# kelseyicotton/rawaudiovae_kelsey

Hardware: AMD Instinct MI355X
Metric: audio frames/sec (fwd+bwd+step), 1024-sample frames (higher is better)
Workload: dtype bf16; 1 GPU; C2 raw-audio VAE train step: S=1024 H=2048 L=64, per-GPU batch 4096, kl_beta=1e-4, Adam lr=1e-4; global_batch=4096, parallelism=dp1, launch=eager, wgrad_slabs=fp16

## Files before the change

rawaudiovae_kelsey_amd/csrc/gemm_bf16.h:

```cpp
#pragma once
#include <type_traits>

#include "common.h"
#include "philox.h"

namespace rv {

enum : int {
  EPI_BIAS_ACT_BF16 = 0,
  EPI_F32 = 1,
  EPI_TANH_LOSS = 2,
  EPI_MASK_BF16 = 3,
  EPI_REPARAM = 4,
  EPI_REPARAM_BWD = 5,
};

struct GemmArgs {
  const bf16_t* A;
  const bf16_t* B;
  long lda, ldb;
  int k_tiles;
  int tiles_m, tiles_n;
  int splits;
  int M_valid, N_valid;
  int relu;
  float* out_f32;
  long ld_f32, split_stride_f32;
  void* out_f16;
  float* f16_unscale;
  long us_ld, us_split_stride;
  bf16_t* out_bf16;
  long ld_bf16;
  const float* bias;
  const bf16_t* mask;
  long ld_mask;
  int mask_fp8;
  const float* x;
  long ld_x;
// ... 20 lines not shown
  float* eps_out;
  unsigned long long seed;
  const long long* step_counter;
  float* mulv;
  bf16_t* z;
  float* kl_partial;
  const float* eps;
  float kl_beta, inv_nk;
  const float* dmu_ext;
  const float* dlv_ext;
  bf16_t* dmulv;
  float* dbh_partial;
  int wt;
};

template <int ROWS>
__device__ __forceinline__ int swz_mn(int k) {
  if constexpr (ROWS >= 128)
    return (k & 3) | (((k >> 3) & 1) << 2);
  else
    return ((k >> 1) & 1) | (((k >> 3) & 1) << 1);
}

__device__ __forceinline__ int swz_mn8(int k) { return ((k >> 1) & 3) | (((k >> 4) & 1) << 2); }

template <int ROWS, bool KMAJ, int NW, bool F8MN = false>
struct StageOffsets {
  static constexpr int NINSTR = ROWS * 128 / 1024;
  static constexpr int PER_WAVE = NINSTR / NW;
  static_assert(NINSTR % NW == 0, "tile must split evenly over the waves");
// ... 119 lines not shown
  }
}

__device__ __forceinline__ unsigned long long pack_fp8x8(const float (&v)[8]) {
  float c[8];
#pragma unroll
  for (int e = 0; e < 8; ++e) c[e] = fminf(fmaxf(v[e], -448.f), 448.f);
  unsigned lo = 0, hi = 0;
  lo = __builtin_amdgcn_cvt_pk_fp8_f32(c[0], c[1], lo, false);
  lo = __builtin_amdgcn_cvt_pk_fp8_f32(c[2], c[3], lo, true);
  hi = __builtin_amdgcn_cvt_pk_fp8_f32(c[4], c[5], hi, false);
  hi = __builtin_amdgcn_cvt_pk_fp8_f32(c[6], c[7], hi, true);
  return ((unsigned long long)hi << 32) | lo;
}

template <int GL>
__device__ __forceinline__ void wait_tiles_in_flight(int tiles) {
  if (tiles >= 6) asm volatile("s_waitcnt vmcnt(%0)" ::"n"(6 * GL < 63 ? 6 * GL : 63) : "memory");
  else if (tiles == 5) asm volatile("s_waitcnt vmcnt(%0)" ::"n"(5 * GL < 63 ? 5 * GL : 63) : "memory");
  else if (tiles == 4) asm volatile("s_waitcnt vmcnt(%0)" ::"n"(4 * GL < 63 ? 4 * GL : 63) : "memory");
  else if (tiles == 3) asm volatile("s_waitcnt vmcnt(%0)" ::"n"(3 * GL) : "memory");
  else if (tiles == 2) asm volatile("s_waitcnt vmcnt(%0)" ::"n"(2 * GL) : "memory");
  else if (tiles == 1) asm volatile("s_waitcnt vmcnt(%0)" ::"n"(GL) : "memory");
  else asm volatile("s_waitcnt vmcnt(0)" ::: "memory");
}

template <int NW>
__device__ __forceinline__ float block_sum(float v, float* red) {
  v = wave_sum(v);
  const int lane = threadIdx.x & 63, w = threadIdx.x >> 6;
  if (lane == 0) red[w] = v;
  __syncthreads();
  float r = 0.f;
  if (threadIdx.x == 0)
    for (int i = 0; i < NW; ++i) r += red[i];
  __syncthreads();
  return r;
}

struct NoGather {};
template <bool A_KMAJ, bool B_KMAJ, bool FP8, typename Hook, typename BRows = NoGather>
__device__ __forceinline__ void mainloop_pingpong(const bf16_t* __restrict__ Ag, const bf16_t* __restrict__ Bg,
                                                  const long lda, const long ldb, const int nk, lds_char* smem,
                                                  const int wave, const int lane, f32x4 (&acc)[8][4], Hook tail_hook,
                                                  BRows b_rows = BRows{}, const long b_half_gather = 0,
                                                  const bf16_t* __restrict__ Ag_next = nullptr,
                                                  const bf16_t* __restrict__ Bg_next = nullptr, const bool resumed = false) {
  constexpr bool GATHER_B = !std::is_same<BRows, NoGather>::value;
  const bool has_next = Ag_next != nullptr;
  constexpr int HALF = 128 * 128;
  constexpr int BUF = 4 * HALF;
  const int wr = wave >> 2, wc = wave & 3;
  StageOffsets<128, A_KMAJ, 8, FP8 && !A_KMAJ> sa;
  StageOffsets<128, B_KMAJ, 8, FP8 && !B_KMAJ> sb;
  sa.init(lda, wave, lane);
  if constexpr (GATHER_B) sb.init_rows(b_rows, wave, lane);
  else sb.init(ldb, wave, lane);
  const int unit_scale = 0x7F7F7F7F;
  constexpr int KROWS = FP8 ? 128 : 64;
  constexpr int MNH = FP8 ? 64 : 128;
// ... 79 lines not shown
      if (kt + 1 < nk || has_next) asm volatile("s_waitcnt vmcnt(4)" ::: "memory");
    }
    mma(I1{}, I1{}, b1);
    if constexpr (EARLY_B) {
      if (kt + 1 < nk) rd_b(bn, nxt, 0);
    }
    stage_b(0, kt + 2);
    if (kt + 2 < nk || has_next) asm volatile("s_waitcnt vmcnt(2)" ::: "memory");
    else asm volatile("s_waitcnt vmcnt(0)" ::: "memory");
    mma(I1{}, I0{}, bq);
  };

  if (!resumed) {
    stage_a(0, 0); stage_a(1, 0); stage_b(0, 0); stage_b(1, 0);
    stage_b(0, 1);
    if (nk > 1) asm volatile("s_waitcnt vmcnt(2)" ::: "memory");
    else asm volatile("s_waitcnt vmcnt(0)" ::: "memory");
    __builtin_amdgcn_s_barrier();
  }
  if constexpr (EARLY_B) rd_b(b0, smem, 0);
  if (wr == 1) __builtin_amdgcn_s_barrier();
  __builtin_amdgcn_sched_barrier(0);

  for (int kt = 0; kt < nk; kt += 2) {
    if constexpr (EARLY_B) {
      k_tile(kt, smem, smem + BUF, b0, b2);
      k_tile(kt + 1, smem + BUF, smem, b2, b0);
    } else {
      k_tile(kt, smem, smem + BUF, b0, b0);
      k_tile(kt + 1, smem + BUF, smem, b0, b0);
    }
  }
  if (wr == 0) __builtin_amdgcn_s_barrier();
  if constexpr (FP8) asm volatile("s_nop 15\n\ts_nop 15" ::: "memory");
  __builtin_amdgcn_sched_barrier(0);
}

template <int BM, int BN, int WGM, int WGN, bool A_KMAJ, bool B_KMAJ, int EPI, int NSTAGE, bool FP8 = false>
__device__ __forceinline__ void gemm_body(const GemmArgs& p, const int bid, char* smem_generic, const int next_bid = -1,
                                          const bool resumed = false) {
  static_assert(!FP8 || NSTAGE == 8 || (A_KMAJ && B_KMAJ), "fp8 operands: K-major (forward) GEMMs on the ring loop, any layout on the ping-pong loop");
  lds_char* smem = (lds_char*)smem_generic;
  constexpr int NW = WGM * WGN;
  constexpr int A_BYTES = BM * 128, B_BYTES = BN * 128, STAGE = A_BYTES + B_BYTES;
  constexpr int B_OFF = A_BYTES;
  constexpr int WTM = BM / WGM, WTN = BN / WGN, MI = WTM / 16, NI = WTN / 16;
  constexpr int GL = STAGE / 1024 / NW;
  constexpr bool PINGPONG = NSTAGE == 8;
  static_assert(PINGPONG || (NSTAGE >= 2 && NSTAGE <= 7 && (NSTAGE - 1) * GL < 64), "vmcnt is a 6-bit counter");
  static_assert(!PINGPONG || (BM == 256 && BN == 256 && WGM == 2 && WGN == 4), "ping-pong loop: 256x256, 2x4 waves");

  const int tid = threadIdx.x, lane = tid & 63;
  const int wave = __builtin_amdgcn_readfirstlane(tid >> 6);
  const int wm = wave / WGN, wn = wave % WGN;
  const int tiles_n = p.tiles_n, nt = p.tiles_n * p.tiles_m, nwg = nt * p.splits;
  auto locate = [&](const int b_, int& split_, int& tile_m_, int& tile_n_) {
    const int xcd = b_ & 7, q = nwg >> 3, rr = nwg & 7;
    const int item = (xcd < rr ? xcd * (q + 1) : rr * (q + 1) + (xcd - rr) * q) + (b_ >> 3);
    split_ = item / nt;
    const int tid_lin = item - split_ * nt;
    if (((tiles_n | p.tiles_m) & 3) == 0) {
      const int sn = tiles_n >> 2, s4 = tid_lin >> 4, w4 = tid_lin & 15;
      tile_m_ = (s4 / sn) * 4 + (w4 >> 2);
      tile_n_ = (s4 % sn) * 4 + (w4 & 3);
    } else {
      tile_m_ = tid_lin / tiles_n;
      tile_n_ = tid_lin - tile_m_ * tiles_n;
    }
  };
  int split, tile_m, tile_n;
  locate(bid, split, tile_m, tile_n);
  const long m0 = (long)tile_m * BM, n0 = (long)tile_n * BN;
  const long k0 = (long)split * p.k_tiles * 64;
  constexpr int F8S = FP8 ? 2 : 1;
  auto a_origin = [&](const long m_, const long k_) { return A_KMAJ ? p.A + m_ * p.lda + k_ : p.A + (F8S * k_) * p.lda + m_ / F8S; };
  auto b_origin = [&](const long n_, const long k_) { return B_KMAJ ? p.B + n_ * p.ldb + k_ : p.B + (F8S * k_) * p.ldb + n_ / F8S; };
  const bf16_t* Ag = a_origin(m0, k0);
  const bf16_t* Bg = b_origin(n0, k0);
  const bf16_t *Ag_next = nullptr, *Bg_next = nullptr;
  if (next_bid >= 0) {
    int s2, tm2, tn2;
    locate(next_bid, s2, tm2, tn2);
    Ag_next = a_origin((long)tm2 * BM, (long)s2 * p.k_tiles * 64);
    Bg_next = b_origin((long)tn2 * BN, (long)s2 * p.k_tiles * 64);
  }
  const long a_step = A_KMAJ ? 64 : 64 * p.lda;
  const long b_step = B_KMAJ ? 64 : 64 * p.ldb;

  static_assert(NI % 2 == 0, "epilogue pairs column fragments");
  constexpr int NP = NI / 2;
  constexpr int CM = (EPI == EPI_REPARAM_BWD && NSTAGE == 8) ? 1 : NP >= 2 ? 2 : (MI >= 4 ? 4 : MI);
  static_assert(MI % CM == 0, "chunking must divide the wave tile");
  constexpr int CH = CM * NP;
  const int eq = lane >> 4, ej = lane & 15;
  const long colw = n0 + wn * WTN + (eq & 1) * 16 + (eq >> 1) * 8;
  const long roww = m0 + wm * WTM + ej;
  typedef int i32x4_ __attribute__((ext_vector_type(4)));

  constexpr bool PF_ROOM = !PINGPONG && MI * NI <= 16;
  constexpr bool PF_X = EPI == EPI_TANH_LOSS && PF_ROOM;
  constexpr bool PF_MASK = EPI == EPI_MASK_BF16 && PF_ROOM;
  float xpf[CH][8];
  i32x4_ mpf[CH];
  bool pf_on = false;
  if constexpr (PF_X) {
    const bool x_al0 = p.x && !p.x_hop && (p.ld_x & 3) == 0 && ((reinterpret_cast<uintptr_t>(p.x) & 15) == 0);
    if (x_al0 && m0 + BM <= p.M_valid && n0 + BN <= p.N_valid) {
      pf_on = true;
#pragma unroll
      for (int it = 0; it < CH; ++it) {
        const float* xs = p.x + (roww + 16 * (it / NP)) * p.ld_x + colw + 32 * (it % NP);
        const f32x4 lo = *(const f32x4*)xs, hi = *(const f32x4*)(xs + 4);
#pragma unroll
        for (int e = 0; e < 4; ++e) { xpf[it][e] = lo[e]; xpf[it][4 + e] = hi[e]; }
      }
    }
  }
  if constexpr (PF_MASK) {
    if (p.mask) {
      pf_on = true;
#pragma unroll
      for (int it = 0; it < CH; ++it)
        mpf[it] = *(const i32x4_*)(p.mask + (roww + 16 * (it / NP)) * p.ld_mask + colw + 32 * (it % NP));
    }
  }
  constexpr bool PF_RB = EPI == EPI_REPARAM_BWD, PF_RF = EPI == EPI_REPARAM;
  constexpr bool PF_RB_ON = PF_RB && MI == CM;
  constexpr int RF_N = MI * (NI / 2);
  f32x4 rb_m[PF_RB ? CH : 1][2], rb_l[PF_RB ? CH : 1][2], rb_e[PF_RB ? CH : (PF_RF ? RF_N : 1)][2];
  bool rb_vec[PF_RB ? CH : (PF_RF ? RF_N : 1)];
  if constexpr (PF_RB_ON) {
    const long L2p_ = 2 * p.lat_lp, L_ = p.lat_l;
    const bool al = (L_ & 3) == 0 && (reinterpret_cast<uintptr_t>(p.eps) & 15) == 0;
#pragma unroll
    for (int it = 0; it < CH; ++it) {
      const long r_ = roww + 16 * (it / NP), c_ = colw + 32 * (it % NP);
      const float* mp = p.mulv + r_ * L2p_ + c_;
      rb_m[it][0] = *(const f32x4*)mp; rb_m[it][1] = *(const f32x4*)(mp + 4);
      rb_l[it][0] = *(const f32x4*)(mp + p.lat_lp); rb_l[it][1] = *(const f32x4*)(mp + p.lat_lp + 4);
      rb_vec[it] = al && r_ < p.M_valid && c_ + 8 <= L_;
// ... 4 lines not shown
      }
    }
  }
  if constexpr (PF_RF) {
    const long L_ = p.lat_l;
    const bool al = RF_N <= 4 && p.eps_in && (L_ & 3) == 0 && (reinterpret_cast<uintptr_t>(p.eps_in) & 15) == 0;
#pragma unroll
    for (int it = 0; it < RF_N; ++it) {
      const long b_ = m0 + wm * WTM + (it / (NI / 2)) * 16 + (lane & 15);
      const long l_ = (long)tile_n * (BN / 2) + wn * (WTN / 2) + (it % (NI / 2)) * 16 + 4 * (lane >> 4);
      rb_vec[it] = al && b_ < p.M_valid && l_ + 4 <= L_;
      rb_e[it][0] = f32x4{0.f, 0.f, 0.f, 0.f};
      if (rb_vec[it]) rb_e[it][0] = *(const f32x4*)(p.eps_in + b_ * L_ + l_);
    }
  }
  if constexpr (PF_X || PF_MASK || PF_RB || PF_RF) {
    asm volatile("" ::: "memory");
    __builtin_amdgcn_sched_barrier(0);
  }

  f32x4 acc[MI][NI];
#pragma unroll
  for (int mi = 0; mi < MI; ++mi)
#pragma unroll
    for (int ni = 0; ni < NI; ++ni) acc[mi][ni] = f32x4{0.f, 0.f, 0.f, 0.f};

  constexpr bool MASK_LDS = EPI == EPI_MASK_BF16 && PINGPONG;
  static_assert(!MASK_LDS || (WTN == 64 && CH == 2 * CM), "mask through LDS: 128-byte mask rows, as many stores as DMA pieces per chunk");
  constexpr int MK_C0 = 2 * CM * 1024;
  lds_char* mk_lds = smem + wave * (WTM * 128);
  lds_char* mk_lds0 = smem + 2 * (BM + BN) * 128 + wave * MK_C0;
  bool mask_lds = false;
  const char* mk_g = nullptr;
  long mk_pitch8 = 0;
  const bool mask8 = FP8 && MASK_LDS && p.mask_fp8;
  if constexpr (MASK_LDS) {
    if (p.mask) {
      mask_lds = true;
      const int mrow = lane >> 3;
      if (mask8) {
        const int mpc = ((lane & 3) ^ (mrow & 3));
        mk_g = (const char*)p.mask + (m0 + wm * WTM + mrow) * p.ld_mask + n0 + wn * WTN + mpc * 16;
        mk_pitch8 = 8 * p.ld_mask;
      } else {
        const int mpc = (lane & 7) ^ (lane >> 3);
        mk_g = (const char*)(p.mask + (m0 + wm * WTM + mrow) * p.ld_mask + n0 + wn * WTN + mpc * 8);
        mk_pitch8 = 16 * p.ld_mask;
      }
    }
  }
  auto mask_dma = [&](int i0, int i1, lds_char* base) {
#pragma unroll
    for (int i = i0; i < i1; ++i)
      __builtin_amdgcn_global_load_lds((glb_cptr)(mk_g + (long)i * mk_pitch8),
                                       (__attribute__((address_space(3))) void*)(base + (i - i0) * 1024), 16, 0, 0);
  };
  if constexpr (PINGPONG && EPI == EPI_REPARAM) {
    static_assert(B_KMAJ && !FP8, "reparameterisation epilogue: bf16 K-major weights");
    mainloop_pingpong<A_KMAJ, B_KMAJ, FP8>(Ag, p.B + k0, p.lda, p.ldb, p.k_tiles, smem, wave, lane, acc, [&]() {},
        [&](int r) { return (((r >> 4) & 1) * p.lat_lp + (long)tile_n * (BN / 2) + (r >> 5) * 16 + (r & 15)) * p.ldb; }, 64 * p.ldb);
  } else if constexpr (PINGPONG) {
    mainloop_pingpong<A_KMAJ, B_KMAJ, FP8>(Ag, Bg, p.lda, p.ldb, p.k_tiles, smem, wave, lane, acc, [&]() {
      if constexpr (MASK_LDS) {
        if (mask_lds) mask_dma(0, 2 * CM, mk_lds0);
      }
    }, NoGather{}, 0, Ag_next, Bg_next, resumed);
  } else {
  StageOffsets<BM, A_KMAJ, NW> sa;
  StageOffsets<BN, B_KMAJ, NW> sb;
  const bf16_t* Agr = Ag;
  bool gathered = false;
  if constexpr (A_KMAJ && EPI == EPI_BIAS_ACT_BF16 && !FP8) {
    if (p.a_hop) {
      gathered = true;
      Agr = p.A + k0;
      sa.init_rows([&](int r) {
        long row = m0 + r;
        row = row < p.a_rows ? row : p.a_rows - 1;
        return (p.a_idx ? (long)p.a_idx[row] : p.a_first + row) * p.a_hop;
      }, wave, lane);
    }
    if (p.step_inc && bid == 0 && tid == 0) *p.step_inc += 1;
  }
  if (!gathered) sa.init(p.lda, wave, lane);
  const bf16_t* Bgr = Bg;
  if constexpr (EPI == EPI_REPARAM) {
    static_assert(B_KMAJ && WTN % 32 == 0, "reparameterisation epilogue: tiles of BN / 2 latents x 2 heads, wave tiles of whole (mu, logvar) fragment pairs");
    Bgr = p.B + k0;
    sb.init_rows([&](int r) { return (((r >> 4) & 1) * p.lat_lp + (long)tile_n * (BN / 2) + (r >> 5) * 16 + (r & 15)) * p.ldb; }, wave, lane);
  } else {
    sb.init(p.ldb, wave, lane);
  }
  auto copy_out = [&](int kt, const lds_char* slot_) {
    if constexpr (A_KMAJ && EPI == EPI_BIAS_ACT_BF16 && !FP8) {
      if (gathered && p.a_copy && kt % tiles_n == tile_n) {
#pragma unroll
        for (int i = 0; i < StageOffsets<BM, A_KMAJ, NW>::PER_WAVE; ++i) {
          const int t = wave + NW * i;
          const int r = 8 * t + (lane >> 3), c = (lane & 7) ^ ((r >> 1) & 7);
          const bf16x8 v_ = *(const __attribute__((address_space(3))) bf16x8*)(slot_ + t * 1024 + lane * 16);
          store_out16((bf16x8*)(p.a_copy + (m0 + r) * p.ld_copy + (long)kt * 64 + c * 8), v_, p.wt);
        }
      }
    }
  };

  const int nk = p.k_tiles;
#pragma unroll
  for (int s = 0; s < NSTAGE; ++s)
    if (s < nk) {
      sa.stage(Agr + s * a_step, smem + s * STAGE, wave);
      sb.stage(Bgr + s * b_step, smem + s * STAGE + B_OFF, wave);
    }
  wait_tiles_in_flight<GL>(nk - 1 < NSTAGE - 1 ? nk - 1 : NSTAGE - 1);
  __builtin_amdgcn_s_barrier();

  bf16x8 a0[MI], b0[NI], a1[MI], b1[NI];
#pragma unroll
  for (int mi = 0; mi < MI; ++mi) a0[mi] = load_frag<BM, A_KMAJ>(smem, wm * WTM + mi * 16, 0, lane);
#pragma unroll
  for (int ni = 0; ni < NI; ++ni) b0[ni] = load_frag<BN, B_KMAJ>(smem + B_OFF, wn * WTN + ni * 16, 0, lane);

  constexpr int NRD = MI * (A_KMAJ ? 1 : 2) + NI * (B_KMAJ ? 1 : 2);
  constexpr int NMF = MI * NI;

  auto first_half = [&](const lds_char* cur) {
#pragma unroll
    for (int mi = 0; mi < MI; ++mi) a1[mi] = load_frag<BM, A_KMAJ>(cur, wm * WTM + mi * 16, 1, lane);
#pragma unroll
// ... 562 lines not shown
        p.colsum[(long)tile_m * tiles_n * BN + n0 + tid] = s_;
      }
    }
    if constexpr (EPI == EPI_TANH_LOSS) {
      if (p.blocksum) {
        __syncthreads();
        float* red = (float*)smem_generic;
        const float s_ = block_sum<NW>(sq, red);
        if (tid == 0) p.blocksum[tile_m * tiles_n + tile_n] = s_;
      }
    }
  }
}

template <int BM, int BN, int WGM, int WGN, bool A_KMAJ, bool B_KMAJ, int EPI, int NSTAGE, bool FP8 = false>
__global__ void __launch_bounds__(64 * WGM * WGN) gemm_bf16_kernel(const GemmArgs p) {
  extern __shared__ __attribute__((aligned(16))) char smem_dyn[];
  gemm_body<BM, BN, WGM, WGN, A_KMAJ, B_KMAJ, EPI, NSTAGE, FP8>(p, blockIdx.x, smem_dyn);
}

template <bool A_KMAJ, bool B_KMAJ, int EPI>
__global__ void __launch_bounds__(512) gemm_pp_persist_kernel(const GemmArgs p) {
  static_assert(EPI == EPI_BIAS_ACT_BF16, "tile lists: epilogues that do not use LDS");
  extern __shared__ __attribute__((aligned(16))) char smem_dyn[];
  const int nwg = p.tiles_m * p.tiles_n * p.splits, G = (int)gridDim.x;
  bool resumed = false;
  for (int vb = (int)blockIdx.x; vb < nwg; vb += G) {
    gemm_body<256, 256, 2, 4, A_KMAJ, B_KMAJ, EPI, 8>(p, vb, smem_dyn, vb + G < nwg ? vb + G : -1, resumed);
    resumed = true;
  }
}

template <int BM, int BN, int WGM, int WGN, int NSTAGE, bool FP8 = false>
__global__ void __launch_bounds__(64 * WGM * WGN)
gemm_dgrad_wgrad_kernel(const GemmArgs dgrad, const GemmArgs wgrad, const int n_first) {
  extern __shared__ __attribute__((aligned(16))) char smem_dyn[];
  if ((int)blockIdx.x < n_first)
    gemm_body<BM, BN, WGM, WGN, true, false, EPI_MASK_BF16, NSTAGE, FP8>(dgrad, blockIdx.x, smem_dyn);
  else
    gemm_body<BM, BN, WGM, WGN, false, false, EPI_F32, NSTAGE, FP8>(wgrad, blockIdx.x - n_first, smem_dyn);
}

template <int BM, int BN, int WGM, int WGN, int NSTAGE, bool A1, bool B1, int E1, bool A2, bool B2, int E2>
__global__ void __launch_bounds__(64 * WGM * WGN)
gemm_dual_kernel(const GemmArgs first, const GemmArgs second, const int n_first) {
  extern __shared__ __attribute__((aligned(16))) char smem_dyn[];
  if ((int)blockIdx.x < n_first)
    gemm_body<BM, BN, WGM, WGN, A1, B1, E1, NSTAGE>(first, blockIdx.x, smem_dyn);
  else
    gemm_body<BM, BN, WGM, WGN, A2, B2, E2, NSTAGE>(second, blockIdx.x - n_first, smem_dyn);
}

}
```

rawaudiovae_kelsey_amd/csrc/gemm_launch.hip:

```cpp
#include <hip/hip_ext.h>
#include "gemm_bf16.h"
#include "adam.h"
#include "../../include/rawvae_hip.h"
#include "internal.h"

using namespace rv;

namespace rv {
thread_local int rv_store_wt = 0;
}

namespace {

int g_force_tile = -1;
int g_tile_lists = 1;

template <int BM, int BN, int WGM, int WGN, int NSTAGE, bool AK, bool BK, int EPI, bool FP8 = false>
int launch(const GemmArgs& a, long Mp, long Np, int splits, hipStream_t st) {
  constexpr int RING = NSTAGE == 8 ? 2 : NSTAGE;
  constexpr int mask_extra = (NSTAGE == 8 && EPI == EPI_MASK_BF16) ? 8 * 4096 : 0;
  constexpr int smem_max = RING * (BM + BN) * 128 + mask_extra;
  constexpr int stage_bytes = (BM + BN) * 128;
  constexpr int epi_bytes = WGM * BN * 4 + 256;
  const int used = (NSTAGE >= 8 ? RING : (a.k_tiles < RING ? a.k_tiles : RING)) * stage_bytes + mask_extra;
  const int smem = used > epi_bytes ? used : epi_bytes;
  auto kern = gemm_bf16_kernel<BM, BN, WGM, WGN, AK, BK, EPI, NSTAGE, FP8>;
  static std::atomic<unsigned long long> attr_done{0};
  lds_opt_in((const void*)kern, smem_max, attr_done);
  GemmArgs g = a;
  g.wt = rv_store_wt;
  g.tiles_m = (int)(Mp / BM);
  g.tiles_n = (int)(Np / BN);
  g.splits = splits;
  dim3 grid((unsigned)(g.tiles_m * g.tiles_n * splits), 1, 1);
  hipLaunchKernelGGL(kern, grid, dim3(64 * WGM * WGN), smem, st, g);
  RV_CHECK_LAUNCH();
  return RV_OK;
}

template <bool AK, bool BK, int EPI>
int launch_persist(const GemmArgs& a, long Mp, long Np, hipStream_t st) {
  constexpr int smem = 2 * (256 + 256) * 128;
  auto kern = gemm_pp_persist_kernel<AK, BK, EPI>;
  static std::atomic<unsigned long long> attr_done{0};
  lds_opt_in((const void*)kern, smem, attr_done);
  GemmArgs g = a;
  g.wt = rv_store_wt;
  g.tiles_m = (int)(Mp / 256);
  g.tiles_n = (int)(Np / 256);
  g.splits = 1;
// ... 34 lines not shown
    case 0: return launch<64, 64, 2, 2, 4, AK, BK, EPI>(a, Mp, Np, splits, st);
    case 1: return launch<128, 128, 2, 2, 4, AK, BK, EPI>(a, Mp, Np, splits, st);
    case 2: return launch<256, 128, 4, 2, 3, AK, BK, EPI>(a, Mp, Np, splits, st);
    case 4: return launch<128, 128, 2, 4, 4, AK, BK, EPI>(a, Mp, Np, splits, st);
    case 5: return launch<256, 256, 2, 4, 2, AK, BK, EPI>(a, Mp, Np, splits, st);
    case 7:
      if ((Kp / 64 / splits) % 2) return launch<256, 256, 2, 4, 2, AK, BK, EPI>(a, Mp, Np, splits, st);
      if constexpr (EPI == EPI_BIAS_ACT_BF16) {
        if (g_tile_lists && splits == 1 && !a.amax_part && !a.a_hop && (Mp / 256) * (Np / 256) >= 512) return launch_persist<AK, BK, EPI>(a, Mp, Np, st);
      }
      return launch<256, 256, 2, 4, 8, AK, BK, EPI>(a, Mp, Np, splits, st);
    default: return launch<256, 128, 2, 2, 3, AK, BK, EPI>(a, Mp, Np, splits, st);
  }
}

template <int NSTAGE, bool FP8 = false>
__global__ void __launch_bounds__(512)
gemm_wgrad_adam_kernel(const GemmArgs wgrad, const int n_gemm, const DescTable tab, float* __restrict__ param,
                       float* __restrict__ m_arena, float* __restrict__ v_arena, const float lr,
                       const float grad_scale, const long long* __restrict__ step_counter, const int stream_mode,
                       float* __restrict__ fin_f32, bf16_t* __restrict__ fin_bf16, const int tail_vb) {
  extern __shared__ __attribute__((aligned(16))) char smem_dyn[];
  if ((int)blockIdx.x < n_gemm) {
    gemm_body<256, 256, 2, 4, false, false, EPI_F32, NSTAGE, FP8>(wgrad, blockIdx.x, smem_dyn);
    if (tail_vb > 0) {
      const long total = tab.blk_start[tab.n];
      const int wave = __builtin_amdgcn_readfirstlane((int)(threadIdx.x >> 6)), lane = (int)(threadIdx.x & 63);
      for (long u = (long)blockIdx.x * 8 + wave; u < 4L * tail_vb; u += 8L * n_gemm)
        adam_block<true>(tab, total - tail_vb + (u >> 2), (int)(u & 3) * 64 + lane, param, m_arena, v_arena, nullptr, lr,
                         grad_scale, step_counter, nullptr, nullptr);
    }
  } else {
    if (fin_f32 || fin_bf16) {
      const long total = tab.blk_start[tab.n];
      const int half = __builtin_amdgcn_readfirstlane((int)(threadIdx.x >> 8));
      for (long vb = 2L * ((long)blockIdx.x - n_gemm) + half; vb < total; vb += 2L * ((long)gridDim.x - n_gemm))
        adam_block<false>(tab, vb, (int)(threadIdx.x & 255), nullptr, nullptr, nullptr, fin_f32, 0.f, 1.f, nullptr, fin_bf16, nullptr);
      return;
    }
    if (stream_mode) {
      const int wave = __builtin_amdgcn_readfirstlane((int)(threadIdx.x >> 6));
      const long n_waves = 8L * ((long)gridDim.x - n_gemm);
      adam_stream(tab, 8L * ((long)blockIdx.x - n_gemm) + wave, n_waves, (lds_char*)smem_dyn + wave * 2 * AS_SLOT,
                  (int)(threadIdx.x & 63), param, m_arena, v_arena, lr, grad_scale, step_counter);
      return;
    }
    const long total = tab.blk_start[tab.n] - tail_vb;
    const long stride = 2L * ((long)gridDim.x - n_gemm);
    const int half = __builtin_amdgcn_readfirstlane((int)(threadIdx.x >> 8));
    constexpr int U = 2;
    for (long vb = 2L * ((long)blockIdx.x - n_gemm) + half; vb < total; vb += U * stride)
      adam_group<U>(tab, vb, stride, (int)(threadIdx.x & 255), param, m_arena, v_arena, lr, grad_scale, step_counter, total);
  }
}

template <int EPI>
int launch_tile_fp8(int tile, const GemmArgs& a, long Mp, long Np, long Kp, hipStream_t st) {
  RV_REQUIRE(Mp > 0 && Np > 0 && Kp > 0 && Kp % 128 == 0, RV_ERR_SHAPE, "fp8 gemm: K must be a multiple of 128 (got %ld)", Kp);
  RV_REQUIRE(tile_fits(tile, Mp, Np), RV_ERR_SHAPE, "fp8 gemm: tile %d does not divide %ld x %ld", tile, Mp, Np);
  switch (tile) {
    case 0: return launch<64, 64, 2, 2, 4, true, true, EPI, true>(a, Mp, Np, 1, st);
    case 2: return launch<256, 128, 4, 2, 3, true, true, EPI, true>(a, Mp, Np, 1, st);
    case 5: case 7: return launch<256, 256, 2, 4, 2, true, true, EPI, true>(a, Mp, Np, 1, st);
    default: return launch<128, 128, 2, 4, 4, true, true, EPI, true>(a, Mp, Np, 1, st);
  }
}

// ... 29 lines not shown

int g_pair_loop = 8;

static thread_local hipEvent_t g_pair_stop_event = nullptr;
template <int NSTAGE, bool FP8 = false>
int launch_pair(const GemmArgs& d_in, const GemmArgs& g_in, hipStream_t st) {
  constexpr int BM = 256, BN = 256, WGM = 2, WGN = 4;
  GemmArgs d = d_in, g = g_in;
  d.wt = g.wt = rv_store_wt;
  const int n_d = d.tiles_m * d.tiles_n, n_w = g.tiles_m * g.tiles_n * g.splits;
  constexpr int smem = 2 * (BM + BN) * 128 + 8 * 4096;
  auto kern = gemm_dgrad_wgrad_kernel<BM, BN, WGM, WGN, NSTAGE, FP8>;
  static std::atomic<unsigned long long> attr_done{0};
  lds_opt_in((const void*)kern, smem, attr_done);
  if (g_pair_stop_event) {
    hipExtLaunchKernelGGL(kern, dim3((unsigned)(n_d + n_w)), dim3(64 * WGM * WGN), smem, st, nullptr, g_pair_stop_event, 0, d, g, n_d);
    g_pair_stop_event = nullptr;
  } else {
    hipLaunchKernelGGL(kern, dim3((unsigned)(n_d + n_w)), dim3(64 * WGM * WGN), smem, st, d, g, n_d);
  }
  RV_CHECK_LAUNCH();
  return RV_OK;
}

template <int BM, int BN, int WGM, int WGN, int NSTAGE, bool A1, bool B1, int E1, bool A2, bool B2, int E2>
int launch_dual(const GemmArgs& a, long Mp1, long Np1, int splits1, const GemmArgs& b, long Mp2, long Np2, int splits2,
                hipStream_t st) {
  constexpr int stage_bytes = (BM + BN) * 128, smem_max = NSTAGE * stage_bytes;
  constexpr int epi_bytes = WGM * BN * 4 + 256;
  const int kt = a.k_tiles > b.k_tiles ? a.k_tiles : b.k_tiles;
  const int used = (kt < NSTAGE ? kt : NSTAGE) * stage_bytes;
  const int smem = used > epi_bytes ? used : epi_bytes;
  auto kern = gemm_dual_kernel<BM, BN, WGM, WGN, NSTAGE, A1, B1, E1, A2, B2, E2>;
  static std::atomic<unsigned long long> attr_done{0};
// ... 272 lines not shown
  const int n_gemm = g.tiles_m * g.tiles_n * splits;
  constexpr int smem = 2 * (256 + 256) * 128;
  static_assert(8 * 2 * AS_SLOT <= smem, "the optimizer waves' LDS rings live in the launch's dynamic LDS");
  int stream_mode = 1;
  for (int i = 0; i < n_desc; ++i)
    if (descs[i].grad_half) stream_mode = 0;
  int tail_vb = 0;
  if (!t.grad_out && !stream_mode) tail_vb = (int)(tab.blk_start[n_desc] * (fp8 ? TAIL_PCT_FP8 : TAIL_PCT_BF16) / 100);
  float* fin_f32 = t.out_bf16 ? nullptr : (float*)t.grad_out;
  bf16_t* fin_bf16 = t.out_bf16 ? (bf16_t*)t.grad_out : nullptr;
  const bool pp = g.k_tiles % 2 == 0;
  const int which = fp8 ? 2 : (pp ? 1 : 0);
  auto kern = fp8 ? gemm_wgrad_adam_kernel<8, true> : (pp ? gemm_wgrad_adam_kernel<8, false> : gemm_wgrad_adam_kernel<2, false>);
  static std::atomic<unsigned long long> attr_done[3];
  lds_opt_in((const void*)kern, smem, attr_done[which]);
  hipLaunchKernelGGL(kern, dim3((unsigned)(n_gemm + n_rider_blocks)), dim3(512), smem, (hipStream_t)stream, g, n_gemm, tab,
                     t.param, t.exp_avg, t.exp_avg_sq, t.lr, t.grad_scale, t.step_counter, stream_mode, fin_f32, fin_bf16, tail_vb);
  RV_CHECK_LAUNCH();
  return RV_OK;
}

extern "C" int rv_pair_stop_event(void* ev) {
  const int pending = g_pair_stop_event != nullptr;
  g_pair_stop_event = (hipEvent_t)ev;
  return pending;
}

extern "C" int rv_linear_wgrad_adam(const void* dy, long lddy, const void* x, long ldx, long Mp, long Np, long Kp, int splits,
                         void* dw, long lddw, int slab_dtype, float* slab_unscale, const rv_param_desc* descs, int n_desc,
                         float* param, float* exp_avg,
                         float* exp_avg_sq, float lr, float grad_scale, const long long* step_counter,
                         int n_adam_blocks, void* stream) {
// ... 148 lines not shown
```

Before: 23.21 million frames/s.

## Issue first GEMM tile loads before epilogue prefetch and accumulator setup

GemmArgs is split into a head and a tail, and the head fields are passed as separate kernel arguments so the mainloop's operand pointers and tile counts sit first in the kernarg segment. Stage-0 A/B loads (and the ping-pong prologue loads) are now issued before the epilogue prefetch of x or mask, the step counter update, accumulator zeroing and mask setup. The waitcnt budget is raised to cover the extra prefetch loads. The aim is to shorten kernel start-up latency for every GEMM tile, at the cost of more complex launch signatures and vmcnt accounting that must stay exact.

Result: no change. 23.17 million frames/s (-0.2%).

```diff
diff --git a/rawaudiovae_kelsey_amd/csrc/gemm_bf16.h b/rawaudiovae_kelsey_amd/csrc/gemm_bf16.h
--- a/rawaudiovae_kelsey_amd/csrc/gemm_bf16.h
+++ b/rawaudiovae_kelsey_amd/csrc/gemm_bf16.h
@@ -15,13 +15,22 @@
   EPI_REPARAM_BWD = 5,
 };
 
-struct GemmArgs {
+struct GemmHead {
   const bf16_t* A;
   const bf16_t* B;
   long lda, ldb;
   int k_tiles;
   int tiles_m, tiles_n;
   int splits;
+  int a_gather;
+};
+#define RV_GEMM_HEAD_PARAMS(x)                                                                                            \
+  const bf16_t *x##A, const bf16_t *x##B, const long x##lda, const long x##ldb, const int x##k_tiles, const int x##tiles_m, \
+      const int x##tiles_n, const int x##splits, const int x##a_gather
+#define RV_GEMM_HEAD_OF(x) GemmHead{x##A, x##B, x##lda, x##ldb, x##k_tiles, x##tiles_m, x##tiles_n, x##splits, x##a_gather}
+#define RV_GEMM_HEAD_ARGS(g) (g).A, (g).B, (g).lda, (g).ldb, (g).k_tiles, (g).tiles_m, (g).tiles_n, (g).splits, (g).a_gather
+
+struct GemmTail {
   int M_valid, N_valid;
   int relu;
   float* out_f32;
@@ -72,6 +81,9 @@
   int wt;
 };
 
+struct GemmArgs : GemmHead, GemmTail {};
+inline const GemmTail& gemm_tail(const GemmArgs& g) { return g; }
+
 template <int ROWS>
 __device__ __forceinline__ int swz_mn(int k) {
   if constexpr (ROWS >= 128)
@@ -221,15 +233,15 @@
   return ((unsigned long long)hi << 32) | lo;
 }
 
-template <int GL>
+template <int GL, int EXTRA = 0>
 __device__ __forceinline__ void wait_tiles_in_flight(int tiles) {
-  if (tiles >= 6) asm volatile("s_waitcnt vmcnt(%0)" ::"n"(6 * GL < 63 ? 6 * GL : 63) : "memory");
-  else if (tiles == 5) asm volatile("s_waitcnt vmcnt(%0)" ::"n"(5 * GL < 63 ? 5 * GL : 63) : "memory");
-  else if (tiles == 4) asm volatile("s_waitcnt vmcnt(%0)" ::"n"(4 * GL < 63 ? 4 * GL : 63) : "memory");
-  else if (tiles == 3) asm volatile("s_waitcnt vmcnt(%0)" ::"n"(3 * GL) : "memory");
-  else if (tiles == 2) asm volatile("s_waitcnt vmcnt(%0)" ::"n"(2 * GL) : "memory");
-  else if (tiles == 1) asm volatile("s_waitcnt vmcnt(%0)" ::"n"(GL) : "memory");
-  else asm volatile("s_waitcnt vmcnt(0)" ::: "memory");
+  if (tiles >= 6) asm volatile("s_waitcnt vmcnt(%0)" ::"n"(6 * GL + EXTRA < 63 ? 6 * GL + EXTRA : 63) : "memory");
+  else if (tiles == 5) asm volatile("s_waitcnt vmcnt(%0)" ::"n"(5 * GL + EXTRA < 63 ? 5 * GL + EXTRA : 63) : "memory");
+  else if (tiles == 4) asm volatile("s_waitcnt vmcnt(%0)" ::"n"(4 * GL + EXTRA < 63 ? 4 * GL + EXTRA : 63) : "memory");
+  else if (tiles == 3) asm volatile("s_waitcnt vmcnt(%0)" ::"n"(3 * GL + EXTRA < 63 ? 3 * GL + EXTRA : 63) : "memory");
+  else if (tiles == 2) asm volatile("s_waitcnt vmcnt(%0)" ::"n"(2 * GL + EXTRA < 63 ? 2 * GL + EXTRA : 63) : "memory");
+  else if (tiles == 1) asm volatile("s_waitcnt vmcnt(%0)" ::"n"(GL + EXTRA < 63 ? GL + EXTRA : 63) : "memory");
+  else asm volatile("s_waitcnt vmcnt(%0)" ::"n"(EXTRA < 63 ? EXTRA : 63) : "memory");
 }
 
 template <int NW>
@@ -246,11 +258,11 @@
 }
 
 struct NoGather {};
-template <bool A_KMAJ, bool B_KMAJ, bool FP8, typename Hook, typename BRows = NoGather>
+template <bool A_KMAJ, bool B_KMAJ, bool FP8, typename Hook, typename HeadHook, typename BRows = NoGather>
 __device__ __forceinline__ void mainloop_pingpong(const bf16_t* __restrict__ Ag, const bf16_t* __restrict__ Bg,
                                                   const long lda, const long ldb, const int nk, lds_char* smem,
                                                   const int wave, const int lane, f32x4 (&acc)[8][4], Hook tail_hook,
-                                                  BRows b_rows = BRows{}, const long b_half_gather = 0,
+                                                  HeadHook head_hook, BRows b_rows = BRows{}, const long b_half_gather = 0,
                                                   const bf16_t* __restrict__ Ag_next = nullptr,
                                                   const bf16_t* __restrict__ Bg_next = nullptr, const bool resumed = false) {
   constexpr bool GATHER_B = !std::is_same<BRows, NoGather>::value;
@@ -360,6 +372,11 @@
   if (!resumed) {
     stage_a(0, 0); stage_a(1, 0); stage_b(0, 0); stage_b(1, 0);
     stage_b(0, 1);
+  }
+  __builtin_amdgcn_sched_barrier(0);
+  head_hook();
+  __builtin_amdgcn_sched_barrier(0);
+  if (!resumed) {
     if (nk > 1) asm volatile("s_waitcnt vmcnt(2)" ::: "memory");
     else asm volatile("s_waitcnt vmcnt(0)" ::: "memory");
     __builtin_amdgcn_s_barrier();
@@ -383,7 +400,7 @@
 }
 
 template <int BM, int BN, int WGM, int WGN, bool A_KMAJ, bool B_KMAJ, int EPI, int NSTAGE, bool FP8 = false>
-__device__ __forceinline__ void gemm_body(const GemmArgs& p, const int bid, char* smem_generic, const int next_bid = -1,
+__device__ __forceinline__ void gemm_body(const GemmHead& h, const GemmTail& p, const int bid, char* smem_generic, const int next_bid = -1,
                                           const bool resumed = false) {
   static_assert(!FP8 || NSTAGE == 8 || (A_KMAJ && B_KMAJ), "fp8 operands: K-major (forward) GEMMs on the ring loop, any layout on the ping-pong loop");
   lds_char* smem = (lds_char*)smem_generic;
@@ -399,13 +416,13 @@
   const int tid = threadIdx.x, lane = tid & 63;
   const int wave = __builtin_amdgcn_readfirstlane(tid >> 6);
   const int wm = wave / WGN, wn = wave % WGN;
-  const int tiles_n = p.tiles_n, nt = p.tiles_n * p.tiles_m, nwg = nt * p.splits;
+  const int tiles_n = h.tiles_n, nt = h.tiles_n * h.tiles_m, nwg = nt * h.splits;
   auto locate = [&](const int b_, int& split_, int& tile_m_, int& tile_n_) {
     const int xcd = b_ & 7, q = nwg >> 3, rr = nwg & 7;
     const int item = (xcd < rr ? xcd * (q + 1) : rr * (q + 1) + (xcd - rr) * q) + (b_ >> 3);
-    split_ = item / nt;
+    split_ = h.splits == 1 ? 0 : item / nt;
     const int tid_lin = item - split_ * nt;
-    if (((tiles_n | p.tiles_m) & 3) == 0) {
+    if (((tiles_n | h.tiles_m) & 3) == 0) {
       const int sn = tiles_n >> 2, s4 = tid_lin >> 4, w4 = tid_lin & 15;
       tile_m_ = (s4 / sn) * 4 + (w4 >> 2);
       tile_n_ = (s4 % sn) * 4 + (w4 & 3);
@@ -417,21 +434,21 @@
   int split, tile_m, tile_n;
   locate(bid, split, tile_m, tile_n);
   const long m0 = (long)tile_m * BM, n0 = (long)tile_n * BN;
-  const long k0 = (long)split * p.k_tiles * 64;
+  const long k0 = (long)split * h.k_tiles * 64;
   constexpr int F8S = FP8 ? 2 : 1;
-  auto a_origin = [&](const long m_, const long k_) { return A_KMAJ ? p.A + m_ * p.lda + k_ : p.A + (F8S * k_) * p.lda + m_ / F8S; };
-  auto b_origin = [&](const long n_, const long k_) { return B_KMAJ ? p.B + n_ * p.ldb + k_ : p.B + (F8S * k_) * p.ldb + n_ / F8S; };
+  auto a_origin = [&](const long m_, const long k_) { return A_KMAJ ? h.A + m_ * h.lda + k_ : h.A + (F8S * k_) * h.lda + m_ / F8S; };
+  auto b_origin = [&](const long n_, const long k_) { return B_KMAJ ? h.B + n_ * h.ldb + k_ : h.B + (F8S * k_) * h.ldb + n_ / F8S; };
   const bf16_t* Ag = a_origin(m0, k0);
   const bf16_t* Bg = b_origin(n0, k0);
   const bf16_t *Ag_next = nullptr, *Bg_next = nullptr;
   if (next_bid >= 0) {
     int s2, tm2, tn2;
     locate(next_bid, s2, tm2, tn2);
-    Ag_next = a_origin((long)tm2 * BM, (long)s2 * p.k_tiles * 64);
-    Bg_next = b_origin((long)tn2 * BN, (long)s2 * p.k_tiles * 64);
-  }
-  const long a_step = A_KMAJ ? 64 : 64 * p.lda;
-  const long b_step = B_KMAJ ? 64 : 64 * p.ldb;
+    Ag_next = a_origin((long)tm2 * BM, (long)s2 * h.k_tiles * 64);
+    Bg_next = b_origin((long)tn2 * BN, (long)s2 * h.k_tiles * 64);
+  }
+  const long a_step = A_KMAJ ? 64 : 64 * h.lda;
+  const long b_step = B_KMAJ ? 64 : 64 * h.ldb;
 
   static_assert(NI % 2 == 0, "epilogue pairs column fragments");
   constexpr int NP = NI / 2;
@@ -446,9 +463,11 @@
   constexpr bool PF_ROOM = !PINGPONG && MI * NI <= 16;
   constexpr bool PF_X = EPI == EPI_TANH_LOSS && PF_ROOM;
   constexpr bool PF_MASK = EPI == EPI_MASK_BF16 && PF_ROOM;
+  constexpr int PF_N = PF_X ? 2 * CH : (PF_MASK ? CH : 0);
   float xpf[CH][8];
   i32x4_ mpf[CH];
   bool pf_on = false;
+  auto prefetch_head = [&]() {
   if constexpr (PF_X) {
     const bool x_al0 = p.x && !p.x_hop && (p.ld_x & 3) == 0 && ((reinterpret_cast<uintptr_t>(p.x) & 15) == 0);
     if (x_al0 && m0 + BM <= p.M_valid && n0 + BN <= p.N_valid) {
@@ -470,6 +489,7 @@
         mpf[it] = *(const i32x4_*)(p.mask + (roww + 16 * (it / NP)) * p.ld_mask + colw + 32 * (it % NP));
     }
   }
+  };
   constexpr bool PF_RB = EPI == EPI_REPARAM_BWD, PF_RF = EPI == EPI_REPARAM;
   constexpr bool PF_RB_ON = PF_RB && MI == CM;
   constexpr int RF_N = MI * (NI / 2);
@@ -504,16 +524,18 @@
       if (rb_vec[it]) rb_e[it][0] = *(const f32x4*)(p.eps_in + b_ * L_ + l_);
     }
   }
-  if constexpr (PF_X || PF_MASK || PF_RB || PF_RF) {
+  if constexpr (PF_RB || PF_RF) {
     asm volatile("" ::: "memory");
     __builtin_amdgcn_sched_barrier(0);
   }
 
   f32x4 acc[MI][NI];
-#pragma unroll
-  for (int mi = 0; mi < MI; ++mi)
-#pragma unroll
-    for (int ni = 0; ni < NI; ++ni) acc[mi][ni] = f32x4{0.f, 0.f, 0.f, 0.f};
+  auto zero_acc = [&]() {
+#pragma unroll
+    for (int mi = 0; mi < MI; ++mi)
+#pragma unroll
+      for (int ni = 0; ni < NI; ++ni) acc[mi][ni] = f32x4{0.f, 0.f, 0.f, 0.f};
+  };
 
   constexpr bool MASK_LDS = EPI == EPI_MASK_BF16 && PINGPONG;
   static_assert(!MASK_LDS || (WTN == 64 && CH == 2 * CM), "mask through LDS: 128-byte mask rows, as many stores as DMA pieces per chunk");
@@ -524,6 +546,7 @@
   const char* mk_g = nullptr;
   long mk_pitch8 = 0;
   const bool mask8 = FP8 && MASK_LDS && p.mask_fp8;
+  auto mask_setup = [&]() {
   if constexpr (MASK_LDS) {
     if (p.mask) {
       mask_lds = true;
@@ -539,6 +562,11 @@
       }
     }
   }
+  };
+  auto pp_head = [&]() {
+    zero_acc();
+    mask_setup();
+  };
   auto mask_dma = [&](int i0, int i1, lds_char* base) {
 #pragma unroll
     for (int i = i0; i < i1; ++i)
@@ -547,39 +575,38 @@
   };
   if constexpr (PINGPONG && EPI == EPI_REPARAM) {
     static_assert(B_KMAJ && !FP8, "reparameterisation epilogue: bf16 K-major weights");
-    mainloop_pingpong<A_KMAJ, B_KMAJ, FP8>(Ag, p.B + k0, p.lda, p.ldb, p.k_tiles, smem, wave, lane, acc, [&]() {},
-        [&](int r) { return (((r >> 4) & 1) * p.lat_lp + (long)tile_n * (BN / 2) + (r >> 5) * 16 + (r & 15)) * p.ldb; }, 64 * p.ldb);
+    mainloop_pingpong<A_KMAJ, B_KMAJ, FP8>(Ag, h.B + k0, h.lda, h.ldb, h.k_tiles, smem, wave, lane, acc, [&]() {}, pp_head,
+        [&](int r) { return (((r >> 4) & 1) * p.lat_lp + (long)tile_n * (BN / 2) + (r >> 5) * 16 + (r & 15)) * h.ldb; }, 64 * h.ldb);
   } else if constexpr (PINGPONG) {
-    mainloop_pingpong<A_KMAJ, B_KMAJ, FP8>(Ag, Bg, p.lda, p.ldb, p.k_tiles, smem, wave, lane, acc, [&]() {
+    mainloop_pingpong<A_KMAJ, B_KMAJ, FP8>(Ag, Bg, h.lda, h.ldb, h.k_tiles, smem, wave, lane, acc, [&]() {
       if constexpr (MASK_LDS) {
         if (mask_lds) mask_dma(0, 2 * CM, mk_lds0);
       }
-    }, NoGather{}, 0, Ag_next, Bg_next, resumed);
+    }, pp_head, NoGather{}, 0, Ag_next, Bg_next, resumed);
   } else {
   StageOffsets<BM, A_KMAJ, NW> sa;
   StageOffsets<BN, B_KMAJ, NW> sb;
   const bf16_t* Agr = Ag;
   bool gathered = false;
   if constexpr (A_KMAJ && EPI == EPI_BIAS_ACT_BF16 && !FP8) {
-    if (p.a_hop) {
+    if (h.a_gather) {
       gathered = true;
-      Agr = p.A + k0;
+      Agr = h.A + k0;
       sa.init_rows([&](int r) {
         long row = m0 + r;
         row = row < p.a_rows ? row : p.a_rows - 1;
         return (p.a_idx ? (long)p.a_idx[row] : p.a_first + row) * p.a_hop;
       }, wave, lane);
     }
-    if (p.step_inc && bid == 0 && tid == 0) *p.step_inc += 1;
-  }
-  if (!gathered) sa.init(p.lda, wave, lane);
+  }
+  if (!gathered) sa.init(h.lda, wave, lane);
   const bf16_t* Bgr = Bg;
   if constexpr (EPI == EPI_REPARAM) {
     static_assert(B_KMAJ && WTN % 32 == 0, "reparameterisation epilogue: tiles of BN / 2 latents x 2 heads, wave tiles of whole (mu, logvar) fragment pairs");
-    Bgr = p.B + k0;
-    sb.init_rows([&](int r) { return (((r >> 4) & 1) * p.lat_lp + (long)tile_n * (BN / 2) + (r >> 5) * 16 + (r & 15)) * p.ldb; }, wave, lane);
+    Bgr = h.B + k0;
+    sb.init_rows([&](int r) { return (((r >> 4) & 1) * p.lat_lp + (long)tile_n * (BN / 2) + (r >> 5) * 16 + (r & 15)) * h.ldb; }, wave, lane);
   } else {
-    sb.init(p.ldb, wave, lane);
+    sb.init(h.ldb, wave, lane);
   }
   auto copy_out = [&](int kt, const lds_char* slot_) {
     if constexpr (A_KMAJ && EPI == EPI_BIAS_ACT_BF16 && !FP8) {
@@ -595,14 +622,26 @@
     }
   };
 
-  const int nk = p.k_tiles;
-#pragma unroll
-  for (int s = 0; s < NSTAGE; ++s)
+  const int nk = h.k_tiles;
+  sa.stage(Agr, smem, wave);
+  sb.stage(Bgr, smem + B_OFF, wave);
+  asm volatile("" ::: "memory");
+  __builtin_amdgcn_sched_barrier(0);
+  prefetch_head();
+  if constexpr (A_KMAJ && EPI == EPI_BIAS_ACT_BF16 && !FP8) {
+    if (p.step_inc && bid == 0 && tid == 0) *p.step_inc += 1;
+  }
+  asm volatile("" ::: "memory");
+  __builtin_amdgcn_sched_barrier(0);
+#pragma unroll
+  for (int s = 1; s < NSTAGE; ++s)
     if (s < nk) {
       sa.stage(Agr + s * a_step, smem + s * STAGE, wave);
       sb.stage(Bgr + s * b_step, smem + s * STAGE + B_OFF, wave);
     }
-  wait_tiles_in_flight<GL>(nk - 1 < NSTAGE - 1 ? nk - 1 : NSTAGE - 1);
+  zero_acc();
+  if (PF_N > 0 && pf_on) wait_tiles_in_flight<GL, PF_N>(nk - 1 < NSTAGE - 1 ? nk - 1 : NSTAGE - 1);
+  else wait_tiles_in_flight<GL>(nk - 1 < NSTAGE - 1 ? nk - 1 : NSTAGE - 1);
   __builtin_amdgcn_s_barrier();
 
   bf16x8 a0[MI], b0[NI], a1[MI], b1[NI];
@@ -1195,9 +1234,16 @@
 }
 
 template <int BM, int BN, int WGM, int WGN, bool A_KMAJ, bool B_KMAJ, int EPI, int NSTAGE, bool FP8 = false>
-__global__ void __launch_bounds__(64 * WGM * WGN) gemm_bf16_kernel(const GemmArgs p) {
+__device__ __forceinline__ void gemm_body(const GemmArgs& p, const int bid, char* smem_generic, const int next_bid = -1,
+                                          const bool resumed = false) {
+  gemm_body<BM, BN, WGM, WGN, A_KMAJ, B_KMAJ, EPI, NSTAGE, FP8>(static_cast<const GemmHead&>(p), static_cast<const GemmTail&>(p), bid,
+                                                                 smem_generic, next_bid, resumed);
+}
+
+template <int BM, int BN, int WGM, int WGN, bool A_KMAJ, bool B_KMAJ, int EPI, int NSTAGE, bool FP8 = false>
+__global__ void __launch_bounds__(64 * WGM * WGN) gemm_bf16_kernel(RV_GEMM_HEAD_PARAMS(h_), const GemmTail p) {
   extern __shared__ __attribute__((aligned(16))) char smem_dyn[];
-  gemm_body<BM, BN, WGM, WGN, A_KMAJ, B_KMAJ, EPI, NSTAGE, FP8>(p, blockIdx.x, smem_dyn);
+  gemm_body<BM, BN, WGM, WGN, A_KMAJ, B_KMAJ, EPI, NSTAGE, FP8>(RV_GEMM_HEAD_OF(h_), p, blockIdx.x, smem_dyn);
 }
 
 template <bool A_KMAJ, bool B_KMAJ, int EPI>
@@ -1214,12 +1260,13 @@
 
 template <int BM, int BN, int WGM, int WGN, int NSTAGE, bool FP8 = false>
 __global__ void __launch_bounds__(64 * WGM * WGN)
-gemm_dgrad_wgrad_kernel(const GemmArgs dgrad, const GemmArgs wgrad, const int n_first) {
+gemm_dgrad_wgrad_kernel(RV_GEMM_HEAD_PARAMS(d_), const int n_first, RV_GEMM_HEAD_PARAMS(w_), const GemmTail dgrad,
+                        const GemmTail wgrad) {
   extern __shared__ __attribute__((aligned(16))) char smem_dyn[];
   if ((int)blockIdx.x < n_first)
-    gemm_body<BM, BN, WGM, WGN, true, false, EPI_MASK_BF16, NSTAGE, FP8>(dgrad, blockIdx.x, smem_dyn);
+    gemm_body<BM, BN, WGM, WGN, true, false, EPI_MASK_BF16, NSTAGE, FP8>(RV_GEMM_HEAD_OF(d_), dgrad, blockIdx.x, smem_dyn);
   else
-    gemm_body<BM, BN, WGM, WGN, false, false, EPI_F32, NSTAGE, FP8>(wgrad, blockIdx.x - n_first, smem_dyn);
+    gemm_body<BM, BN, WGM, WGN, false, false, EPI_F32, NSTAGE, FP8>(RV_GEMM_HEAD_OF(w_), wgrad, blockIdx.x - n_first, smem_dyn);
 }
 
 template <int BM, int BN, int WGM, int WGN, int NSTAGE, bool A1, bool B1, int E1, bool A2, bool B2, int E2>
diff --git a/rawaudiovae_kelsey_amd/csrc/gemm_launch.hip b/rawaudiovae_kelsey_amd/csrc/gemm_launch.hip
--- a/rawaudiovae_kelsey_amd/csrc/gemm_launch.hip
+++ b/rawaudiovae_kelsey_amd/csrc/gemm_launch.hip
@@ -32,8 +32,9 @@
   g.tiles_m = (int)(Mp / BM);
   g.tiles_n = (int)(Np / BN);
   g.splits = splits;
+  g.a_gather = g.a_hop != 0;
   dim3 grid((unsigned)(g.tiles_m * g.tiles_n * splits), 1, 1);
-  hipLaunchKernelGGL(kern, grid, dim3(64 * WGM * WGN), smem, st, g);
+  hipLaunchKernelGGL(kern, grid, dim3(64 * WGM * WGN), smem, st, RV_GEMM_HEAD_ARGS(g), gemm_tail(g));
   RV_CHECK_LAUNCH();
   return RV_OK;
 }
@@ -98,43 +99,51 @@
   }
 }
 
+struct RiderArgs {
+  float* param;
+  float* m_arena;
+  float* v_arena;
+  float lr, grad_scale;
+  const long long* step_counter;
+  int stream_mode;
+  float* fin_f32;
+  bf16_t* fin_bf16;
+  int tail_vb;
+};
 template <int NSTAGE, bool FP8 = false>
 __global__ void __launch_bounds__(512)
-gemm_wgrad_adam_kernel(const GemmArgs wgrad, const int n_gemm, const DescTable tab, float* __restrict__ param,
-                       float* __restrict__ m_arena, float* __restrict__ v_arena, const float lr,
-                       const float grad_scale, const long long* __restrict__ step_counter, const int stream_mode,
-                       float* __restrict__ fin_f32, bf16_t* __restrict__ fin_bf16, const int tail_vb) {
+gemm_wgrad_adam_kernel(RV_GEMM_HEAD_PARAMS(w_), const int n_gemm, const GemmTail wgrad, const DescTable tab, const RiderArgs ra) {
   extern __shared__ __attribute__((aligned(16))) char smem_dyn[];
   if ((int)blockIdx.x < n_gemm) {
-    gemm_body<256, 256, 2, 4, false, false, EPI_F32, NSTAGE, FP8>(wgrad, blockIdx.x, smem_dyn);
-    if (tail_vb > 0) {
+    gemm_body<256, 256, 2, 4, false, false, EPI_F32, NSTAGE, FP8>(RV_GEMM_HEAD_OF(w_), wgrad, blockIdx.x, smem_dyn);
+    if (ra.tail_vb > 0) {
       const long total = tab.blk_start[tab.n];
       const int wave = __builtin_amdgcn_readfirstlane((int)(threadIdx.x >> 6)), lane = (int)(threadIdx.x & 63);
-      for (long u = (long)blockIdx.x * 8 + wave; u < 4L * tail_vb; u += 8L * n_gemm)
-        adam_block<true>(tab, total - tail_vb + (u >> 2), (int)(u & 3) * 64 + lane, param, m_arena, v_arena, nullptr, lr,
-                         grad_scale, step_counter, nullptr, nullptr);
+      for (long u = (long)blockIdx.x * 8 + wave; u < 4L * ra.tail_vb; u += 8L * n_gemm)
+        adam_block<true>(tab, total - ra.tail_vb + (u >> 2), (int)(u & 3) * 64 + lane, ra.param, ra.m_arena, ra.v_arena, nullptr, ra.lr,
+                         ra.grad_scale, ra.step_counter, nullptr, nullptr);
     }
   } else {
-    if (fin_f32 || fin_bf16) {
+    if (ra.fin_f32 || ra.fin_bf16) {
       const long total = tab.blk_start[tab.n];
       const int half = __builtin_amdgcn_readfirstlane((int)(threadIdx.x >> 8));
       for (long vb = 2L * ((long)blockIdx.x - n_gemm) + half; vb < total; vb += 2L * ((long)gridDim.x - n_gemm))
-        adam_block<false>(tab, vb, (int)(threadIdx.x & 255), nullptr, nullptr, nullptr, fin_f32, 0.f, 1.f, nullptr, fin_bf16, nullptr);
+        adam_block<false>(tab, vb, (int)(threadIdx.x & 255), nullptr, nullptr, nullptr, ra.fin_f32, 0.f, 1.f, nullptr, ra.fin_bf16, nullptr);
       return;
     }
-    if (stream_mode) {
+    if (ra.stream_mode) {
       const int wave = __builtin_amdgcn_readfirstlane((int)(threadIdx.x >> 6));
       const long n_waves = 8L * ((long)gridDim.x - n_gemm);
       adam_stream(tab, 8L * ((long)blockIdx.x - n_gemm) + wave, n_waves, (lds_char*)smem_dyn + wave * 2 * AS_SLOT,
-                  (int)(threadIdx.x & 63), param, m_arena, v_arena, lr, grad_scale, step_counter);
+                  (int)(threadIdx.x & 63), ra.param, ra.m_arena, ra.v_arena, ra.lr, ra.grad_scale, ra.step_counter);
       return;
     }
-    const long total = tab.blk_start[tab.n] - tail_vb;
+    const long total = tab.blk_start[tab.n] - ra.tail_vb;
     const long stride = 2L * ((long)gridDim.x - n_gemm);
     const int half = __builtin_amdgcn_readfirstlane((int)(threadIdx.x >> 8));
     constexpr int U = 2;
     for (long vb = 2L * ((long)blockIdx.x - n_gemm) + half; vb < total; vb += U * stride)
-      adam_group<U>(tab, vb, stride, (int)(threadIdx.x & 255), param, m_arena, v_arena, lr, grad_scale, step_counter, total);
+      adam_group<U>(tab, vb, stride, (int)(threadIdx.x & 255), ra.param, ra.m_arena, ra.v_arena, ra.lr, ra.grad_scale, ra.step_counter, total);
   }
 }
 
@@ -194,10 +203,12 @@
   static std::atomic<unsigned long long> attr_done{0};
   lds_opt_in((const void*)kern, smem, attr_done);
   if (g_pair_stop_event) {
-    hipExtLaunchKernelGGL(kern, dim3((unsigned)(n_d + n_w)), dim3(64 * WGM * WGN), smem, st, nullptr, g_pair_stop_event, 0, d, g, n_d);
+    hipExtLaunchKernelGGL(kern, dim3((unsigned)(n_d + n_w)), dim3(64 * WGM * WGN), smem, st, nullptr, g_pair_stop_event, 0, RV_GEMM_HEAD_ARGS(d), n_d,
+                          RV_GEMM_HEAD_ARGS(g), gemm_tail(d), gemm_tail(g));
     g_pair_stop_event = nullptr;
   } else {
-    hipLaunchKernelGGL(kern, dim3((unsigned)(n_d + n_w)), dim3(64 * WGM * WGN), smem, st, d, g, n_d);
+    hipLaunchKernelGGL(kern, dim3((unsigned)(n_d + n_w)), dim3(64 * WGM * WGN), smem, st, RV_GEMM_HEAD_ARGS(d), n_d, RV_GEMM_HEAD_ARGS(g),
+                       gemm_tail(d), gemm_tail(g));
   }
   RV_CHECK_LAUNCH();
   return RV_OK;
@@ -500,8 +511,9 @@
   auto kern = fp8 ? gemm_wgrad_adam_kernel<8, true> : (pp ? gemm_wgrad_adam_kernel<8, false> : gemm_wgrad_adam_kernel<2, false>);
   static std::atomic<unsigned long long> attr_done[3];
   lds_opt_in((const void*)kern, smem, attr_done[which]);
-  hipLaunchKernelGGL(kern, dim3((unsigned)(n_gemm + n_rider_blocks)), dim3(512), smem, (hipStream_t)stream, g, n_gemm, tab,
-                     t.param, t.exp_avg, t.exp_avg_sq, t.lr, t.grad_scale, t.step_counter, stream_mode, fin_f32, fin_bf16, tail_vb);
+  hipLaunchKernelGGL(kern, dim3((unsigned)(n_gemm + n_rider_blocks)), dim3(512), smem, (hipStream_t)stream, RV_GEMM_HEAD_ARGS(g), n_gemm,
+                     gemm_tail(g), tab,
+                     RiderArgs{t.param, t.exp_avg, t.exp_avg_sq, t.lr, t.grad_scale, t.step_counter, stream_mode, fin_f32, fin_bf16, tail_vb});
   RV_CHECK_LAUNCH();
   return RV_OK;
 }
```
